# Psy-Fer/SquiggleKit

Hardware: AMD Instinct MI355X
Metric: reads/sec MotifSeq DTW (4k-sample read x 200-sample motif) (higher is better)
Workload: dtype f64 results; u32 fixed-point screening

## Files before the change

squigglekit_amd/csrc/sk_prepw_dev.h:

```cpp
#pragma once
#include "sk_common.h"

namespace {

typedef short i16x2 __attribute__((ext_vector_type(2)));

__device__ __forceinline__ unsigned clamp_pk_i16(unsigned q, unsigned lo2, unsigned hi2)
{
    const i16x2 x = __builtin_bit_cast(i16x2, q);
    const i16x2 c = __builtin_elementwise_min(__builtin_elementwise_max(x, __builtin_bit_cast(i16x2, lo2)),
                                              __builtin_bit_cast(i16x2, hi2));
    return __builtin_bit_cast(unsigned, c);
}

__device__ __forceinline__ int wave_incl_scan(int v)
{
    v += __builtin_amdgcn_update_dpp(0, v, 0x111, 0xF, 0xF, false);
    v += __builtin_amdgcn_update_dpp(0, v, 0x112, 0xF, 0xF, false);
    v += __builtin_amdgcn_update_dpp(0, v, 0x114, 0xF, 0xF, false);
    v += __builtin_amdgcn_update_dpp(0, v, 0x118, 0xF, 0xF, false);
    v += __builtin_amdgcn_update_dpp(0, v, 0x142, 0xA, 0xF, false);
    v += __builtin_amdgcn_update_dpp(0, v, 0x143, 0xC, 0xF, false);
    return v;
}
// ... 46 lines not shown
    const unsigned long long own2 = __ballot(local > 0 && k2 >= pre && k2 < pre + local);
    b1 = bcast_from(i1, own1 ? (int)__builtin_ctzll(own1) : 0);
    b2 = bcast_from(i2, own2 ? (int)__builtin_ctzll(own2) : 0);
}

struct prepw_env {
    unsigned *hist;
    int lo, hi, nbins, nb4;
    int hb0;
    bool in_vec, out_vec;
    unsigned lo2, hi2;
};

template <int NQ>
__device__ __forceinline__ prepw_env prepw_setup(unsigned *hist, int lane, int lo, int hi, int vec_ok)
{
    prepw_env e;
    e.hist = hist; e.lo = lo; e.hi = hi;
    e.nbins = hi - lo - 1;
    e.nb4 = (e.nbins + 3) & ~3;
    e.hb0 = lane * 4 * NQ;
    e.in_vec = (vec_ok & 1) != 0; e.out_vec = (vec_ok & 2) != 0;
    const int lo1 = max(lo + 1, -32768), hi1 = min(hi - 1, 32767);
    e.lo2 = (unsigned)(lo1 & 0xffff) * 0x10001u; e.hi2 = (unsigned)(hi1 & 0xffff) * 0x10001u;
#pragma unroll
    for (int j = 0; j < NQ; j++)
        if (e.hb0 + 4 * j < e.nb4) *(uint4 *)(hist + e.hb0 + 4 * j) = make_uint4(0u, 0u, 0u, 0u);
    return e;
}

template <int NQ>
__device__ __forceinline__ sk_prep prepw_read(const prepw_env &E, const int16_t *__restrict__ sig, int64_t stride,
                                              const int32_t *__restrict__ len, int r, int lane,
                                              int16_t *__restrict__ comp, sk_prep *__restrict__ prep)
{
    unsigned *const hist = E.hist;
    unsigned *const hist_v = hist - (E.lo + 1);
    const int lo = E.lo, hi = E.hi, nbins = E.nbins, nb4 = E.nb4, hb0 = E.hb0;
    const bool in_vec = E.in_vec, out_vec = E.out_vec;
    const unsigned lo2 = E.lo2, hi2 = E.hi2;
    auto load8 = [&](const int16_t *row, int M, int i0, unsigned (&q)[4]) {
        if (in_vec && i0 + 8 <= M) {
            const uint4 t = *(const uint4 *)(row + i0);
            q[0] = t.x; q[1] = t.y; q[2] = t.z; q[3] = t.w;
        } else {
#pragma unroll
            for (int k = 0; k < 4; k++) {
                const unsigned a = (i0 + 2 * k < M) ? (unsigned short)row[i0 + 2 * k] : 0u;
                const unsigned b = (i0 + 2 * k + 1 < M) ? (unsigned short)row[i0 + 2 * k + 1] : 0u;
                q[k] = a | (b << 16);
            }
        }
    };
    {
        const int M = min(max(len[r], 0), (int)min(stride, (int64_t)0x7fffff00));
        const int16_t *row = sig + (int64_t)r * stride;
        int16_t *crow = comp + (int64_t)r * stride;

        int run = 0;
        {
            unsigned v[4], vn[4];
            load8(row, M, lane * 8, v);
            for (int base = 0; base < M; base += 512) {
                const int i0 = base + lane * 8;
                if (base + 512 < M) load8(row, M, i0 + 512, vn);
                unsigned changed = 0;
#pragma unroll
// ... 6 lines not shown
                } else {
                    unsigned keep = 0;
#pragma unroll
                    for (int k = 0; k < 8; k++) {
                        const int x = sample_of(v, k);
                        if (i0 + k < M && x > lo && x < hi) keep |= 1u << k;
                    }
                    const int cnt = __popc(keep);
                    const int inc = wave_incl_scan(cnt);
                    int o = run + inc - cnt;
#pragma unroll
                    for (int k = 0; k < 8; k++) {
                        if (keep & (1u << k)) {
                            const int x = sample_of(v, k);
                            crow[o++] = (int16_t)x;
                            atomicAdd(&hist_v[x], 1u);
                        }
                    }
                    run += bcast_from(inc, 63);
                }
#pragma unroll
                for (int k = 0; k < 4; k++) v[k] = vn[k];
            }
        }
        const int n = run;

        sk_prep pr;
        pr.n = n; pr.flags = 0; pr.center = 0.0; pr.scale = 1.0; pr.top = 0.0; pr.bot = 0.0;
        if (n == 0) {
            pr.flags = SK_FLAG_EMPTY;
            const double qnan = __builtin_nan("");
            pr.center = qnan; pr.scale = qnan; pr.top = qnan; pr.bot = qnan;
            if (lane == 0) prep[r] = pr;
            return pr;
        }

        unsigned cnt[4 * NQ];
#pragma unroll
        for (int j = 0; j < NQ; j++) {
            uint4 q = make_uint4(0u, 0u, 0u, 0u);
            if (hb0 + 4 * j < nb4) q = *(const uint4 *)(hist + hb0 + 4 * j);
            cnt[4 * j] = q.x; cnt[4 * j + 1] = q.y; cnt[4 * j + 2] = q.z; cnt[4 * j + 3] = q.w;
        }
        int b1, b2, pre_med;
        rank2<NQ>(cnt, lane, (n - 1) / 2, n / 2, b1, b2, &pre_med);
        const int med2 = (b1 + lo + 1) + (b2 + lo + 1);

        const int odd = med2 & 1;
        const int cl = ((med2 - odd) >> 1) - (lo + 1);
        const int cr = cl + odd;
        {
            int acc = pre_med;
#pragma unroll
            for (int j = 0; j < NQ; j++) {
                uint4 q;
                acc += (int)cnt[4 * j];     q.x = (unsigned)acc;
                acc += (int)cnt[4 * j + 1]; q.y = (unsigned)acc;
                acc += (int)cnt[4 * j + 2]; q.z = (unsigned)acc;
                acc += (int)cnt[4 * j + 3]; q.w = (unsigned)acc;
                if (hb0 + 4 * j < nb4) *(uint4 *)(hist + hb0 + 4 * j) = q;
            }
        }
        auto within = [&](int t) -> int {
            const int hi_i = min(cr + t, nbins - 1), lo_i = cl - t - 1;
            const int a = (int)hist[hi_i];
            const int b = (lo_i >= 0) ? (int)hist[max(lo_i, 0)] : 0;
            return a - b;
        };
        const int k1 = (n - 1) / 2, k2 = n / 2;
        const int step = (nbins + 63) >> 6;
        const int cend = within(lane * step + step - 1);
        const unsigned long long ge1 = __ballot(cend > k1), ge2 = __ballot(cend > k2);
        const int B1 = ge1 ? (int)__builtin_ctzll(ge1) : 63, B2 = ge2 ? (int)__builtin_ctzll(ge2) : 63;
        const int half = lane >> 5, li = lane & 31;
        const int tprobe = (half ? B2 : B1) * step + li;
        const int cin = within(tprobe);
        const unsigned long long hit = __ballot(li < step && cin > (half ? k2 : k1));
        const unsigned h1 = (unsigned)hit, h2 = (unsigned)(hit >> 32);
        const int t1 = B1 * step + (h1 ? (int)__builtin_ctz(h1) : step - 1);
// ... 227 lines not shown
```

squigglekit_amd/csrc/sk_runtime.hip:

```cpp
#include "sk_common.h"
#include <string>
#include <string.h>
#include <mutex>
#include <stdio.h>
#include <stdlib.h>
#include <string.h>

static thread_local char  g_err[512] = "";
static thread_local int   g_cur = -1;
static sk_ctx             g_ctx[SK_MAX_DEVICES];
static std::mutex         g_mu;
static std::recursive_mutex g_ctx_mu[SK_MAX_DEVICES];

int sk_fail(int code, const char *fmt, ...)
{
    va_list ap;
    va_start(ap, fmt);
    vsnprintf(g_err, sizeof g_err, fmt, ap);
    va_end(ap);
    return code;
}

sk_entry::sk_entry() : sk_entry(g_cur) {}

// ... 23 lines not shown
    (void)c;
    if (bytes <= b->cap) return SK_OK;
    if (b->p) { SK_HIP(hipFree(b->p)); b->p = nullptr; b->cap = 0; }
    size_t want = bytes + bytes / 8 + 256;
    hipError_t e = hipMalloc(&b->p, want);
    if (e != hipSuccess) {
        b->p = nullptr;
        return sk_fail(SK_ERR_NOMEM, "hipMalloc(%zu) failed: %s", want, hipGetErrorString(e));
    }
    b->cap = want;
    return SK_OK;
}

int sk_second_stream(sk_ctx *c)
{
    if (!c->stream2) {
        SK_HIP(hipStreamCreateWithFlags(&c->stream2, hipStreamNonBlocking));
        for (int i = 0; i < 9; i++) SK_HIP(hipEventCreateWithFlags(&c->ev_chunk[i], hipEventDisableTiming));
    }
    return SK_OK;
}

struct sk_tunable { const char *name, *test_values, *what; };
static const sk_tunable SK_TUNABLES[] = {
    {"SK_DTW_SCHEME",         "full exact2", "DTW scheme: full = one exact pass, exact2 = two exact passes (default: fixed-point screening + certified window)"},
    {"SK_DTW_QL",             "8 16 64",     "lanes per read of the screening scheme (default: by motif length and batch size)"},
    {"SK_DTW_NOFUSE",         "1",           "filter + medmad as their own kernel instead of the screening pass's prologue"},
    {"SK_DTW_FORCE_RETRY_PM", "100 1000",    "per-mille of reads sent through the exact retry whatever the window pass certified (sensitivity runs)"},
    {"SK_DTW_SPAN",           "150 300",     "look-back of the window pass in columns (one tier)"},
    {"SK_DTW_SPAN2",          "0 500",       "look-back of the window pass's second tier (0: none)"},
    {"SK_DTW_CK",             "64 256",      "steps between checkpoints of the screening pass (multiple of 64)"},
    {"SK_DTW_NOSORT",         "1",           "window passes take the reads in file order"},
    {"SK_DTW_NOHINT",         "1",           "no start hint: the plain screening sweep, every read's exact window looks back the same number of columns"},
    {"SK_DTW_HINT_MIN",       "1",           "the start hint is on for calls of at least this many reads (default 500000)"},
    {"SK_DTW_SORT_MIN",       "1",           "window passes sort chunks of at least this many reads"},
    {"SK_DTW_NO_EARLY",       "1",           "no early exact retry beside the window passes"},
    {"SK_DTW_NO_SIBLINGS",    "1",           "reads whose candidate columns fall into two clusters take the exact pass (no second window)"},
    {"SK_DTW_NOGUARD",        "1",           "screening scheme without its run-time guard (premise test in the window pass, audit, gated exact fallback): A/B cost runs"},
    {"SK_DTW_AUDIT_PERIOD",   "0 1 64",      "the audit re-runs one read in this many with the exact pass (default 4096; 0: no audit)"},
    {"SK_DTW_HOLE",           "qerr1 fma64 fma64x", "tests: a known precision hole put back (E = 1; the fma sample image for float64 reads, with / without the image-error guard) -- the guard has to notice and the records must not change"},
    {"SK_DTW_SCRATCH_MB",     "8 64",        "checkpoint scratch budget in MB (small values force many chunks)"},
    {"SK_DTW_NO_SMALL",       "1",           "small batches keep the batch lane layout"},
    {"SK_DTW_SMALL_MAX",      "0 100000",    "largest batch that spreads a read over 64 lanes"},
    {"SK_PREP_BLOCK",         "1",           "medmad statistics by the workgroup-per-read kernel"},
    {"SK_PREP_ROUNDS",        "1 3",         "grid rounds of the persistent statistics kernels"},
    {"SK_PREP_PERCU",         "1 2",         "workgroups per CU of the persistent statistics kernels"},
    {"SK_SEG_OLD",            "1",           "segmenter: numpy-order statistics kernels for every read"},
    {"SK_SEG_DELTA_SCALE",    "1e13",        "segmenter: certification margin multiplier (large: every read takes the numpy-order redo)"},
    {"SK_SEG_PA_F64",         "1",           "segmenter, raw reads through the pA conversion: expand to float64 and take the float64 kernels instead of the raw-domain kernel"},
    {"SK_SEG_NO_WG",          "1",           "segmenter, reads of 4 097 .. 65 536 samples: the wavefront-per-read statistics kernel (two looks at a read) instead of the workgroup-per-read one"},
    {"SK_SEG_WG_ALL",         "1",           "segmenter: the workgroup-per-read statistics kernel for every row of 4 097 .. 65 536 samples (default: where it is faster)"},
    {"SK_SEG_OCC",            "7 8",         "segmenter statistics kernel: waves per SIMD the registers are sized for"},
    {"SK_SEG_CHUNKS",         "2 8",         "segmenter: chunks of a large batch (walk of one beside the statistics of the next)"},
    {"SK_WALK_GENERAL",       "1",           "segmenter walk: general step (corrector test live)"},
    {"SK_WALK_SYNC",          "1",           "segmenter walk: run hopping with the 64 lanes of a wavefront on the same word (k_seg_walk3)"},
    {"SK_WALK_OWNPASS",       "1",           "segmenter walk: finds the quiet stretches and anchors in a pass of its own instead of taking the statistics kernel's hints"},
    {"SK_WALK_NOJUMP",        "1",           "segmenter walk: every run is hopped through, no jumps between the stretches of quiet entries"},
    {"SK_WALK_NOWAVE",        "1",           "segmenter walk: a lane per read also for long rows / small batches (no wavefront-per-read walk)"},
    {"SK_WALK_WAVE_MAXREADS", "0 1000000",   "segmenter walk: batches of up to this many reads take the wavefront-per-read walk (default: 16384, 131072 for rows beyond 4 096 samples)"},
    {"SK_DRNA_STEP",          "1",           "dRNA_segmenter, both branches: the per-sample scans instead of the scans by runs / by transitions"},
    {"SK_ROLL_TWO_KERNELS",   "1",           "dRNA_segmenter rolling-mean branch: filter kernel + prefix sums through HBM instead of the one-look kernel (prefix sums in LDS)"},
    {"SK_ROLL_ONE_LOOK",      "1",           "dRNA_segmenter rolling-mean branch: the workgroup-per-read kernel in numpy's order for every read instead of the streaming kernel with certified thresholds"},
    {"SK_ROLL_DELTA_SCALE",   "1e13",        "dRNA_segmenter rolling-mean branch: multiplier of the certification margin (large: every read is redone in numpy's order)"},
    {"SK_HITS_ROW_BYTES",     "1000000",     "hit lists: bytes of the last-row buffer (12 B per column and read; default 2 GiB; small values force many chunks of reads)"},
    {"SK_PANEL_EXACT",        "1",           "motif panel: the one-grid exact kernel also for long windows over many reads (default: those take the screening scheme, one launch set per motif)"},
    {"SK_PATH_LDS_BYTES",     "0",           "alignment paths: bytes of direction words a hit may keep in LDS (default and most 25600; 0: every hit takes the scratch tier)"},
// ... 308 lines not shown
```

squigglekit_amd/csrc/sk_sdtwq.hip:

```cpp
#include "sk_sdtw_dev.h"
#include "sk_prepw_dev.h"
#include <math.h>
#include <stdlib.h>
#include <string.h>
#include <vector>

#ifndef SK_SDTWQ_FEED
#define SK_SDTWQ_FEED 0
#define SK_SDTWQ_MAIN 1
#endif

namespace {

template <int R>
__device__ __forceinline__ void qcolumn(const unsigned (&old)[R], unsigned (&nw)[R], const unsigned (&xq)[R],
                                        unsigned yq, unsigned dg, unsigned up)
{
    constexpr int R4 = R & ~3;
#pragma unroll
    for (int k = 0; k < R4; k += 4) {
        asm("v_min3_u32 %0, %12, %4, %13\n\t"
            "v_sad_u32 %0, %8, %14, %0 clamp\n\t"
            "v_min3_u32 %1, %4, %5, %0\n\t"
            "v_sad_u32 %1, %9, %14, %1 clamp\n\t"
// ... 98 lines not shown
    const unsigned *ls = a.lsum + (int64_t)(r - a.read0) * (a.nck + 1) * L + l;
    const unsigned thr = (b > QINF - 2u * a.qerr) ? QINF : b + 2u * a.qerr;
    int hs = 0x7fffffff;
    for (int cc = jlo / a.ck; cc <= min(a.nck, (jhi + L - 1) / a.ck); cc++) {
        if (ls[(int64_t)cc * L] > thr) continue;
        const int j0 = cc * a.ck + l - (L - 1);
        for (int q = 0; q < a.ck / L; q++) {
            const int j = j0 + q * L;
            if (j < jlo || j > jhi) continue;
            const unsigned w = lastq[j + L];
            if (w > thr) continue;
            const int gj = j >> HINT_G;
            const int gs = gj - (int)((unsigned)(gj - (int)(w & HINT_MASK)) & HINT_MASK);
            hs = min(hs, max(gs, 0) << HINT_G);
        }
    }
#pragma unroll
    for (int d = 1; d < L; d <<= 1) hs = min(hs, __shfl_xor(hs, d));
    return hs;
}

#ifndef SK_Q_WAVES
#define SK_Q_WAVES(R) 4
#endif
#ifdef SK_SDTWQ_HINT
#define SK_Q_KERNEL k_sdtw_qh
#define SK_P_KERNEL k_sdtw_ph
constexpr bool HINT = true;
#else
#define SK_Q_KERNEL k_sdtw_q
#define SK_P_KERNEL k_sdtw_p
constexpr bool HINT = false;
#endif
template <int L, int R, int FEED, bool P0>
__global__ __launch_bounds__(256) __attribute__((amdgpu_waves_per_eu(SK_Q_WAVES(R), 8)))
void SK_Q_KERNEL(const sdtw_kargs a)
{
    static_assert(L == 8 || L == 16 || L == 64, "lanes per read");
    static_assert(!HINT || (FEED == SK_FEED_I16 && L <= (1 << HINT_G) && (1 << HINT_G) % L == 0),
                  "tagged sweep: int16 feed, a block of L steps inside one granule");
    constexpr int G = 64 / L;
    constexpr int CKH = (R + 3) / 2;
    constexpr int U = (L < 16) ? L : 16;

    const int lane = threadIdx.x & 63;
    const int wave = blockIdx.x * (blockDim.x >> 6) + (threadIdx.x >> 6);
    const int g = lane / L, l = lane % L;
    int slot = wave * G + g;
    const bool live = slot < a.nreads;
    if (!live) slot = a.nreads - 1;
    const int r = a.read0 + slot;
    const bool timer = a.clk && blockIdx.x == 0 && threadIdx.x < 64;
    unsigned long long tc0 = 0, tr0 = 0;
    if (timer) { tc0 = __builtin_amdgcn_s_memtime(); tr0 = __builtin_amdgcn_s_memrealtime(); }

    extern __shared__ __align__(16) unsigned char lds_dyn[];
    __shared__ __align__(16) unsigned lds_all[4][5 * 64];
    int n;
    double center = 0.0, scale = 1.0;
    const int16_t *s16 = nullptr;
    const double  *s64 = nullptr;
    if constexpr (FEED == SK_FEED_I16) {
        if (a.fz_raw) {
            unsigned *wlds = (unsigned *)lds_dyn + (size_t)(threadIdx.x >> 6) * a.lds_wave_words;
            n = 0;
            if (a.fz_mode == 0) {
                const prepw_env E = prepw_setup<5>(wlds, lane, a.fz_lo, a.fz_hi, a.fz_vec);
                for (int gg = 0; gg < G; gg++) {
                    if (wave * G + gg >= a.nreads) break;
                    const sk_prep pr = prepw_read<5>(E, a.fz_raw, a.stride, a.fz_len, a.read0 + wave * G + gg, lane,
                                                     (int16_t *)a.samples, (sk_prep *)a.prep);
                    if (g == gg) { n = pr.n; center = pr.center; scale = pr.scale; }
                }
            } else {
                const zs_env E = zs_setup((int16_t *)wlds, (double *)lds_all[threadIdx.x >> 6], a.fz_lo, a.fz_hi, a.fz_vec);
#pragma unroll 1
                for (int gg = 0; gg < G; gg++) {
                    if (wave * G + gg >= a.nreads) break;
                    const sk_prep pr = zs_read(E, a.fz_raw, a.stride, a.fz_len, a.read0 + wave * G + gg, lane,
                                               (int16_t *)a.samples, (sk_prep *)a.prep);
                    if (g == gg) { n = pr.n; center = pr.center; scale = pr.scale; }
                    __builtin_amdgcn_wave_barrier();
                }
            }
            __builtin_amdgcn_fence(__ATOMIC_RELEASE, "workgroup");
            __builtin_amdgcn_fence(__ATOMIC_ACQUIRE, "workgroup");
        } else {
            const sk_prep pr = a.prep[r];
            n = pr.n; center = pr.center; scale = pr.scale;
        }
        s16 = (const int16_t *)a.samples + (int64_t)r * a.stride;
    } else if constexpr (FEED == SK_FEED_F64_NORM) {
        const sk_prep pr = a.prep[r];
        n = pr.n; center = pr.center; scale = pr.scale;
        s64 = (const double *)(((pr.flags & SK_IFLAG_INPLACE) && a.samples_raw) ? a.samples_raw : a.samples) + a.off[r];
    } else {
        n = (int)(a.off[r + 1] - a.off[r]);
        s64 = (const double *)a.samples + a.off[r];
    }
    if (!live) n = 0;
    const double inv_scale = 1.0 / scale;

    int nsteps = (n > 0) ? n - 1 + L : 0;
#pragma unroll
    for (int d = L; d < 64; d <<= 1) nsteps = max(nsteps, __shfl_xor(nsteps, d));
// ... 7 lines not shown
    const unsigned notfirst = (l == 0) ? 0u : 0xffffffffu;
    [[maybe_unused]] unsigned tagv = 0;

    unsigned Da[R], Db[R];
#pragma unroll
    for (int k = 0; k < R; k++) { Da[k] = QINF; Db[k] = QINF; }
    unsigned botq = (R == 1 && l == 0 && shortlane) ? 0u : QINF;
    unsigned diagq = (l == 0) ? 0u : QINF;
    int bad = 0;
    if constexpr (FEED == SK_FEED_F64_NORM) {
        if (live && (a.prep[r].flags & SK_FLAG_RECENTRE)) bad = 1;
    }
    unsigned qmin = QINF;
    unsigned smin = QINF;

    const int nlast = max(n - 1, 0);
    if (n == 0) { s16 = (const int16_t *)a.xlayq; s64 = (const double *)a.xlayq; }
    auto loadraw = [&](int idx) {
        if constexpr (FEED == SK_FEED_I16) return (int)s16[min(idx, nlast)];
        else                               return s64[min(idx, nlast)];
    };
    const double qa = inv_scale * QSCALE, qb = -center * qa;
    const bool fma64 = FEED == SK_FEED_F64_NORM && a.hole >= SK_HOLE_FMA64;
    if (live && n > 0) {
        double imgerr = 0.0;
        if (FEED == SK_FEED_I16 || fma64)            imgerr = 3.8e-7 + fabs(center) * qa * 1.2e-16;
        else if constexpr (FEED == SK_FEED_F64_NORM) imgerr = 5.7e-7;
        const bool rej = !(imgerr * (double)(HINT ? a.qplen : a.qerr) <= 1.0) && a.hole != SK_HOLE_FMA64_UNGUARDED;
        if (rej) {
            bad = 1;
            if (l == 0 && a.guard) atomicAdd(&a.guard[SK_GUARD_IMGREJ], 1);
        }
    }
    auto toq = [&](auto raw_, int idx) -> unsigned {
        const double raw = (double)raw_;
        double t;
        if constexpr (FEED == SK_FEED_I16)           t = __builtin_fma(raw, qa, qb);
        else if constexpr (FEED == SK_FEED_F64_NORM) t = fma64 ? __builtin_fma(raw, qa, qb) : (raw - center) * qa;
        else                                         t = raw * QSCALE;
        const bool ok = fabs(t) < QLIM * QSCALE;
        unsigned q = (unsigned)__double2loint(t + 6755399441055744.0) ^ 0x80000000u;
        if constexpr (HINT) q &= ~HINT_MASK;
        const bool in = idx < n;
        bad |= (in && !ok) ? 1 : 0;
        return (in && ok) ? q : QINF;
    };

    const unsigned smask = shortlane ? 0xffffffffu : 0u;
    unsigned *lastq = a.lastq + (int64_t)(r - a.read0) * a.lq_stride;
    unsigned *ybuf = lds_all[threadIdx.x >> 6] + g * 5 * L;
    unsigned *dump = ybuf + 3 * L;
    unsigned *ibuf = (unsigned *)lds_dyn + (size_t)(threadIdx.x >> 6) * a.lds_wave_words + g * a.ck;
    int ioff = 0;
    unsigned gmin = QINF;
    ybuf[L + l] = QINF;
    unsigned F = toq(loadraw(l), l);
    auto step = [&](const unsigned (&old)[R], unsigned (&nw)[R], unsigned yq, unsigned *hslot) {
        unsigned upq;
        if constexpr (HINT) upq = shrtag<L>(botq, tagv);
        else                upq = shr0<L>(botq, notfirst);
        qcolumn<R>(old, nw, xq, yq, diagq, upq);
        diagq = upq;
        if constexpr (P0)          botq = nw[R - 1];
        else if constexpr (R >= 2) asm("v_bitop3_b32 %0, %1, %2, %3 bitop3:0xe4" : "=v"(botq) : "v"(nw[R - 2]), "v"(nw[R - 1]), "v"(smask));
        else                       asm("v_bitop3_b32 %0, %1, %2, %3 bitop3:0xe4" : "=v"(botq) : "v"(upq), "v"(nw[0]), "v"(smask));
        *hslot = nw[R - 1];
    };
    auto flush = [&](int c, int nb) {
        unsigned im = smin;
#pragma unroll
        for (int d = 1; d < L; d <<= 1) im = min(im, (unsigned)__shfl_xor((int)im, d));
        const unsigned lim = (gmin > QINF - 2u * a.qerr) ? QINF : gmin + 2u * a.qerr;
        const bool keep = live && im <= lim;
        gmin = min(gmin, im);
        if (keep) {
            unsigned *dst = lastq + (int64_t)c * a.ck + l + 1;
            for (int q = 0; q < nb; q++) dst[q * L] = ibuf[q * L + l];
        }
// ... 220 lines not shown
            }
            const unsigned Fnext = toq(t0 + L + l);
            const unsigned *yr;
            if (pb & 1) { ybuf[L + l] = Fq; yr = ybuf + L - l; }
            else        { ybuf[l] = Fq; ybuf[2 * L + l] = Fq; yr = ybuf + 2 * L - l; }
#pragma unroll 1
            for (int q = 0; q < L; q += 2) {
                const unsigned y0 = yr[q], y1 = yr[q + 1];
                qstep(Qs, Qn, y0);
                qstep(Qn, Qs, y1);
            }
            Fq = Fnext;
        }
    }
    if (c0 > 0 && npre == 0) load_ckpt();
    tbase += npre * L;

    if (live) {
        if (c0 > 0) {
            unsigned *ws = a.wstate + ((int64_t)slot * L + l) * CKW;
#pragma unroll
            for (int k = 0; k < R; k++) ws[k] = Qs[k];
            ws[R] = botq; ws[R + 1] = diagq;
        }
        if (l == 0) {
            wrec w;
            w.tbase = tbase; w.jlo = jlo; w.jhi = jhi;
            w.flags = (screened ? 1 : 0) | (c0 > 0 ? 2 : 0) | clustered;
            ((wrec *)a.wrec)[slot] = w;
        }
    }
}

template <int L, int R, int FEED>
__global__ __launch_bounds__(256) __attribute__((amdgpu_waves_per_eu(R <= 13 ? 4 : (R <= 26 ? 3 : 2), 8)))
void k_sdtw_w(const sdtw_kargs a)
{
    constexpr int G = 64 / L;
    constexpr bool XLDS = R > 16;
    constexpr int SHR = (L == 64) ? DPP_WAVE_SHR1 : DPP_ROW_SHR1;
    constexpr int CKW = R + 2;
    constexpr int U = (L < 16) ? L : 8;
    const double INF = __builtin_huge_val();

    const int lane = threadIdx.x & 63;
    const int wave = blockIdx.x * (blockDim.x >> 6) + (threadIdx.x >> 6);
    const int g = lane / L, l = lane % L;
    int slot = wave * G + g;
    int nreads = a.nreads;
    if (a.wl_count) {
        nreads = min(*a.wl_count, a.nreads);
        if (nreads <= 0) return;
    }
    const bool live = slot < nreads;
    if (!live) slot = nreads - 1;
    const int r = a.tier2 == 2 ? ((const sibrec *)a.sib)[slot].r : a.wl_list ? a.wl_list[slot] : a.read0 + slot;

    int n, flags = 0;
    double center = 0.0, scale = 1.0;
    const int16_t *s16 = nullptr;
    const double  *s64 = nullptr;
    if constexpr (FEED == SK_FEED_I16) {
        const sk_prep pr = a.prep[r];
        n = pr.n; flags = pr.flags & SK_FLAG_PUBLIC; center = pr.center; scale = pr.scale;
        s16 = (const int16_t *)a.samples + (int64_t)r * a.stride;
    } else if constexpr (FEED == SK_FEED_F64_NORM) {
        const sk_prep pr = a.prep[r];
        n = pr.n; flags = pr.flags & SK_FLAG_PUBLIC; center = pr.center; scale = pr.scale;
        s64 = (const double *)(((pr.flags & SK_IFLAG_INPLACE) && a.samples_raw) ? a.samples_raw : a.samples) + a.off[r];
    } else {
// ... 88 lines not shown
#pragma unroll
            for (int q = 0; q < U; q++) {
                const int t = tbase + blk * L + qq + q;
                const double y = yv[q];
                double upD;  int upS;
                if constexpr (L >= 16) {
                    upD = dpp_f64<SHR>(0.0, botD);
                    upS = dpp_i32<SHR>(t + 1, botS);
                } else {
                    const unsigned lo = shr0<L>((unsigned)__double2loint(botD), notfirst);
                    const unsigned hi = shr0<L>((unsigned)__double2hiint(botD), notfirst);
                    upD = __hiloint2double((int)hi, (int)lo);
                    upS = (int)(shr0<L>((unsigned)botS, notfirst) | (first & (unsigned)(t + 1)));
                }
                double dgD = diagD;  int dgS = diagS;
                double uD = upD;     int uS = upS;
#pragma unroll
                for (int k = 0; k < R; k++) {
                    const double lfD = D[k];  const int lfS = S[k];
                    const double xk = XLDS ? xl[k] : x[k];
                    const double c = fabs(xk - y);
                    const bool lt1 = lfD < dgD;
                    const double m1 = vmin(lfD, dgD);
                    const int    s1 = lt1 ? lfS : dgS;
                    const bool lt2 = uD < m1;
                    const double m = vmin(uD, m1);
                    const int    s = lt2 ? uS : s1;
                    const double nd = c + m;
                    dgD = lfD;  dgS = lfS;
                    D[k] = nd;  S[k] = s;
                    uD = nd;    uS = s;
                }
                diagD = upD;  diagS = upS;
                if constexpr (R >= 2) {
                    botD = shortlane ? D[R - 2] : D[R - 1];
                    botS = shortlane ? S[R - 2] : S[R - 1];
                } else {
                    botD = shortlane ? upD : D[0];
                    botS = shortlane ? upS : S[0];
                }
                if (blk * L + qq + q >= s0) {
                    const int j = t - l;
                    if (j >= jlo && j <= jhi && D[R - 1] < best) { best = D[R - 1]; bestS = S[R - 1]; bestJ = j; }
                }
            }
        }
        F = Fnext;
    }

    auto premise_holds = [&](double bestD, int j) -> bool {
        if (!a.guard) return true;
        const unsigned lq = a.lastq[(int64_t)(r - a.read0) * a.lq_stride + j + L];
        const unsigned bq = (unsigned)a.qflag[r - a.read0];
        const double u = bestD * QSCALE, e = (double)a.qerr;
        const double e2 = (rec.flags & 4) ? 3.0 * e : e;
        const bool ok = fabs(u - (double)lq) <= e && u <= (double)bq + e2;
        if (!ok) { atomicAdd(&a.guard[SK_GUARD_VIOL], 1); atomicAdd(&a.guard[SK_GUARD_ALARM], 1); }
        return ok;
    };
    if (live && l == L - 1) {
        sk_hit h;
        h.n = n; h.flags = flags;
        const bool forced = a.force_retry && (((unsigned)r * 2654435761u) >> 22) < (unsigned)a.force_retry;
        bool certified = false;
        if (a.tier2 == 2) {
            h.dist = best; h.start = bestS; h.end = bestJ;
            h.n = (n > 0 && screened && bestS >= 0 && !forced && premise_holds(best, bestJ)) ? 1 : 0;
            a.sib_out[slot] = h;
        } else if (n <= 0) {
            h.dist = __builtin_nan(""); h.start = -1; h.end = -1;
            a.out[r] = h;
        } else if (screened && bestS >= 0 && !forced && (certified = premise_holds(best, bestJ))) {
            h.dist = best; h.start = bestS; h.end = bestJ;
            a.out[r] = h;
        } else if (!screened && a.early_cnt && !a.tier2) {
        } else {
            h.dist = __builtin_nan(""); h.start = -1; h.end = -1;
            a.out[r] = h;
            const bool violated = screened && bestS >= 0 && !forced && !certified;
            if (screened && a.soft && !forced && !violated) a.soft[atomicAdd(a.soft_cnt, 1)] = r;
            else                                            a.retry[atomicAdd(a.retry_cnt, 1)] = r;
        }
    }
}

typedef void (*sdtw_fn)(const sdtw_kargs);

template <int L, int FEED, int WHICH>
sdtw_fn pick_r(int R)
{
#ifndef SK_SDTWQ_HINT
#define SK_KERNEL(RR) (WHICH == 0 ? (sdtw_fn)SK_Q_KERNEL<L, RR, FEED, false> :     \
                       WHICH == 3 ? (sdtw_fn)SK_Q_KERNEL<L, RR, FEED, (RR >= 2)> : \
                       WHICH == 1 ? (sdtw_fn)SK_P_KERNEL<L, RR, FEED> : (sdtw_fn)k_sdtw_w<L, RR, FEED>)
#else
#define SK_KERNEL(RR) (WHICH == 0 ? (sdtw_fn)SK_Q_KERNEL<L, RR, FEED, false> :     \
                       WHICH == 3 ? (sdtw_fn)SK_Q_KERNEL<L, RR, FEED, (RR >= 2)> : (sdtw_fn)SK_P_KERNEL<L, RR, FEED>)
#endif
    switch (R) { SK_R_CASES_1_16(SK_KERNEL) }
    if constexpr (L != 64) {
        switch (R) { SK_R_CASES_17_32(SK_KERNEL) }
    }
#undef SK_KERNEL
    return nullptr;
}

template <int WHICH, int FEED>
sdtw_fn pick_l(int L, int R)
{
    if (L == 8)  return pick_r<8, FEED, WHICH>(R);
    if (L == 16) return pick_r<16, FEED, WHICH>(R);
#ifndef SK_SDTWQ_HINT
    return pick_r<64, FEED, WHICH>(R);
#else
    return nullptr;
#endif
}

}

#if defined(SK_SDTWQ_HINT)
void *sk_sdtwq_pick_hint(int which, int L, int R)
#elif SK_SDTWQ_FEED == 0
void *sk_sdtwq_pick_feed0(int which, int L, int R)
#elif SK_SDTWQ_FEED == 1
void *sk_sdtwq_pick_feed1(int which, int L, int R)
#else
void *sk_sdtwq_pick_feed2(int which, int L, int R)
#endif
{
    switch (which) {
    case 0: return (void *)pick_l<0, SK_SDTWQ_FEED>(L, R);
    case 1: return (void *)pick_l<1, SK_SDTWQ_FEED>(L, R);
    case 3: return (void *)pick_l<3, SK_SDTWQ_FEED>(L, R);
#ifndef SK_SDTWQ_HINT
    default: return (void *)pick_l<2, SK_SDTWQ_FEED>(L, R);
#else
    default: return nullptr;
#endif
    }
}

#ifdef SK_SDTWQ_MAIN
void *sk_sdtwq_pick_feed1(int which, int L, int R);
void *sk_sdtwq_pick_feed2(int which, int L, int R);
void *sk_sdtwq_pick_hint(int which, int L, int R);

static void screen_layout(int N, int64_t nreads, int64_t maxlen, int *L, int *R)
{
    int l = (N <= 8 * 32 && nreads >= (maxlen > 8192 ? 65536 : 49152)) ? 8 : (N <= 16 * 32) ? 16 : 64;
    if (const char *e = sk_tune("SK_DTW_QL")) {
        const int v = atoi(e);
        if ((v == 8 && N <= 8 * 32) || (v == 16 && N <= 16 * 32) || v == 64) l = v;
    }
    *L = l;
    *R = (N + l - 1) / l;
}

constexpr int ORDER_BINS = 1024;

struct order_args {
    const wrec    *rec;
    const int32_t *qflag;
    int nreads, read0, span, ck, nck, L, wmax;
    int hint;
    int32_t *hist;
    int32_t *order;
};

__device__ __forceinline__ int order_key(const order_args &a, int i)
{
    const wrec q = a.rec[i];
    const unsigned b = (unsigned)a.qflag[i];
    if (!((b < QSAFE) && (q.jhi >= q.jlo) && (q.jhi - q.jlo <= a.wmax))) return ORDER_BINS - 1;
    const int tx = a.hint ? min(max(q.tbase, 0), q.jlo) : max(0, q.jlo - a.span);
    int c0 = tx / a.ck;
    if (c0 > a.nck) c0 = a.nck;
    const int npre = c0 > 0 ? (tx - c0 * a.ck) / a.L : 0;
    const int tbase = c0 * a.ck + npre * a.L;
// ... 111 lines not shown
    int64_t chunk;
    while (true) {
        chunk = sk_dtw_chunk_reads(per_read, a->nreads);
        rc = sk_reserve(c, &c->ckpt, (size_t)chunk * (size_t)(nck > 0 ? nck : 1) * ck_bytes);
        if (!rc) rc = sk_reserve(c, &c->lastq, (size_t)chunk * lq_stride * sizeof(unsigned));
        if (!rc) rc = sk_reserve(c, &c->wstate, (size_t)chunk * state_bytes);
        if (!rc) rc = sk_reserve(c, &c->lsum, (size_t)chunk * (size_t)(nck + 1) * L * sizeof(unsigned));
        if (rc != SK_ERR_NOMEM || chunk <= 1024) break;
        sk_dtw_scratch_shrink(0);
    }
    if (rc) return rc;
    if ((rc = sk_reserve(c, &c->qflag, (size_t)chunk * sizeof(int32_t)))) return rc;
    if ((rc = sk_reserve(c, &c->wrec, (size_t)chunk * sizeof(wrec)))) return rc;
    if ((rc = sk_reserve(c, &c->wrecq, (size_t)chunk * sizeof(wrec)))) return rc;
    int sort_min = 32768;
    if (const char *e = sk_tune("SK_DTW_SORT_MIN")) { const int v = atoi(e); if (v > 0) sort_min = v; }
    const bool sorted = chunk >= sort_min && sk_tune("SK_DTW_NOSORT") == nullptr;
    if (sorted && (rc = sk_reserve(c, &c->order, ((size_t)chunk + ORDER_BINS) * sizeof(int32_t)))) return rc;
    const bool tiers = span2 > span;
    if (tiers && (rc = sk_reserve(c, &c->wsoft, ((size_t)chunk + 1) * sizeof(int32_t)))) return rc;
    const bool siblings = sk_tune("SK_DTW_NO_SIBLINGS") == nullptr;
    const int sib_cap = (int)(chunk / 64 + 1024);
    if (siblings) {
        if ((rc = sk_reserve(c, &c->sib, 16 + (size_t)sib_cap * sizeof(sibrec)))) return rc;
        if ((rc = sk_reserve(c, &c->sibout, (size_t)sib_cap * sizeof(sk_hit)))) return rc;
        if ((rc = sk_reserve(c, &c->sibstate, (size_t)sib_cap * (state_bytes + sizeof(wrec))))) return rc;
        if (c->stream3 && !c->ev_s[0])
            for (int i = 0; i < 2; i++) SK_HIP(hipEventCreateWithFlags(&c->ev_s[i], hipEventDisableTiming));
    }

    typedef void *(*pick_fn)(int, int, int);
    const pick_fn pk = a->feed == SK_FEED_I16 ? (pick_fn)sk_sdtwq_pick_feed0
                     : a->feed == SK_FEED_F64_NORM ? (pick_fn)sk_sdtwq_pick_feed1 : (pick_fn)sk_sdtwq_pick_feed2;
    sdtw_fn fq = (sdtw_fn)pk(P == 0 ? 3 : 0, L, R), fp = (sdtw_fn)pk(1, L, R), fw = (sdtw_fn)pk(2, L, R);
    const int64_t plen = (int64_t)N + maxlen + 2;
    int64_t hint_min = HINT_MIN_READS;
    if (const char *e = sk_tune("SK_DTW_HINT_MIN")) { const int v = atoi(e); if (v > 0) hint_min = v; }
    const bool hint = a->feed == SK_FEED_I16 && (L == 8 || L == 16) && plen <= HINT_MAX_PLEN && R <= HINT_MAX_R &&
                      a->nreads >= hint_min && sk_tune("SK_DTW_NOHINT") == nullptr;
    sdtw_fn fp1 = fp;
    if (hint) { fq = (sdtw_fn)sk_sdtwq_pick_hint(P == 0 ? 3 : 0, L, R); fp1 = (sdtw_fn)sk_sdtwq_pick_hint(1, L, R); }
    if (!fq || !fp || !fp1 || !fw) return sk_fail(SK_ERR_UNSUPPORTED, "no screening kernel for L=%d R=%d", L, R);

    sdtw_kargs k = kargs_of(a);
    k.xlay = (const double *)c->motifw.p; k.xlayq = (const unsigned *)c->motifq.p; k.P = P; k.out = a->out;
    k.nck = nck; k.ck = ck; k.span = span; k.retry = d_retry; k.retry_cnt = d_retry_cnt;
    k.ckq = (unsigned *)c->ckpt.p; k.lastq = (unsigned *)c->lastq.p; k.lq_stride = (int64_t)lq_stride;
    k.qflag = (int32_t *)c->qflag.p; k.lsum = (unsigned *)c->lsum.p;
    k.wstate = (unsigned *)c->wstate.p; k.wrec = c->wrec.p; k.wrec_q = c->wrecq.p;
    k.early_cnt = d_early_cnt; k.early = d_early;
    k.qplen = (unsigned)plen;
    k.qerr = hint ? ((unsigned)plen << HINT_T) + HINT_MASK : (unsigned)plen;
    k.wmax = 4 * ck;
    k.lds_wave_words = (64 / L) * ck;
    k.guard = sk_tune("SK_DTW_NOGUARD") ? nullptr : (int32_t *)c->dtwcnt.p + 8;
    k.wsteps = (unsigned long long *)((char *)c->dtwcnt.p + 64);
    if (const char *e = sk_tune("SK_DTW_HOLE")) {
        k.hole = strcmp(e, "qerr1") == 0 ? SK_HOLE_QERR1 : strcmp(e, "fma64") == 0 ? SK_HOLE_FMA64
               : strcmp(e, "fma64x") == 0 ? SK_HOLE_FMA64_UNGUARDED : SK_HOLE_NONE;
        if (k.hole == SK_HOLE_QERR1) k.qerr = 1;
    }
    if (const char *e = sk_tune("SK_DTW_FORCE_RETRY_PM")) {
        const int pm = atoi(e);
        if (pm > 0) k.force_retry = pm >= 1000 ? 1024 : (pm * 1024 + 999) / 1000;
    }

    size_t fz_lds = 0;
    const sk_prep_fuse fz = a->fuse ? *a->fuse : sk_prep_fuse();
    if (a->fuse) {
        const int need = fz.mode == SK_PREP_ZSCALE ? (int)((a->stride * 2 + 15) / 16 * 4) : (((fz.hi - fz.lo - 1) + 3) & ~3);
        if (need > k.lds_wave_words) k.lds_wave_words = need;
    }
    fz_lds = (size_t)4 * (size_t)k.lds_wave_words * sizeof(unsigned);
    if (fz_lds + 5 * 1024 > 64 * 1024)
// ... 99 lines not shown
```

Measured before the change: 17.48 million.

## Hoist fixed-point range test to per-read value range from fused prologue

The fused int16 filter+medmad prologue now reports each read's min and max sample value, taken from the histogram. The screening kernel checks the fixed-point overflow bound once per read on those two ends, so the per-sample range test and bad-flag update leave the hot conversion. A window-kernel variant for P==0 also reads the bottom row directly instead of selecting on shortlane. This adds new template instantiations and a separate compile unit, and the per-read test is only valid because quantization is monotone in the raw value.

```diff
diff --git a/squigglekit_amd/csrc/sk_prepw_dev.h b/squigglekit_amd/csrc/sk_prepw_dev.h
--- a/squigglekit_amd/csrc/sk_prepw_dev.h
+++ b/squigglekit_amd/csrc/sk_prepw_dev.h
@@ -102,7 +102,8 @@
 template <int NQ>
 __device__ __forceinline__ sk_prep prepw_read(const prepw_env &E, const int16_t *__restrict__ sig, int64_t stride,
                                               const int32_t *__restrict__ len, int r, int lane,
-                                              int16_t *__restrict__ comp, sk_prep *__restrict__ prep)
+                                              int16_t *__restrict__ comp, sk_prep *__restrict__ prep,
+                                              int (*vrange)[2] = nullptr)
 {
     unsigned *const hist = E.hist;
     unsigned *const hist_v = hist - (E.lo + 1);
@@ -175,6 +176,7 @@
             const double qnan = __builtin_nan("");
             pr.center = qnan; pr.scale = qnan; pr.top = qnan; pr.bot = qnan;
             if (lane == 0) prep[r] = pr;
+            if (vrange) { (*vrange)[0] = 0; (*vrange)[1] = 0; }
             return pr;
         }
 
@@ -188,6 +190,16 @@
         int b1, b2, pre_med;
         rank2<NQ>(cnt, lane, (n - 1) / 2, n / 2, b1, b2, &pre_med);
         const int med2 = (b1 + lo + 1) + (b2 + lo + 1);
+        if (vrange) {
+            int first = 4 * NQ, last = -1;
+#pragma unroll
+            for (int i = 4 * NQ - 1; i >= 0; i--) if (cnt[i]) first = i;
+#pragma unroll
+            for (int i = 0; i < 4 * NQ; i++) if (cnt[i]) last = i;
+            const unsigned long long have = __ballot(last >= 0);
+            (*vrange)[0] = bcast_from(hb0 + first, (int)__builtin_ctzll(have)) + lo + 1;
+            (*vrange)[1] = bcast_from(hb0 + last, 63 - (int)__builtin_clzll(have)) + lo + 1;
+        }
 
         const int odd = med2 & 1;
         const int cl = ((med2 - odd) >> 1) - (lo + 1);
diff --git a/squigglekit_amd/csrc/sk_runtime.hip b/squigglekit_amd/csrc/sk_runtime.hip
--- a/squigglekit_amd/csrc/sk_runtime.hip
+++ b/squigglekit_amd/csrc/sk_runtime.hip
@@ -79,6 +79,7 @@
     {"SK_DTW_CK",             "64 256",      "steps between checkpoints of the screening pass (multiple of 64)"},
     {"SK_DTW_NOSORT",         "1",           "window passes take the reads in file order"},
     {"SK_DTW_NOHINT",         "1",           "no start hint: the plain screening sweep, every read's exact window looks back the same number of columns"},
+    {"SK_DTW_RANGE_PER_SAMPLE", "1",         "screening sweep behind the fused filter + medmad prologue: the fixed-point range test on every sample (default there: once per read, on the ends of its value range)"},
     {"SK_DTW_HINT_MIN",       "1",           "the start hint is on for calls of at least this many reads (default 500000)"},
     {"SK_DTW_SORT_MIN",       "1",           "window passes sort chunks of at least this many reads"},
     {"SK_DTW_NO_EARLY",       "1",           "no early exact retry beside the window passes"},
diff --git a/squigglekit_amd/csrc/sk_sdtwq.hip b/squigglekit_amd/csrc/sk_sdtwq.hip
--- a/squigglekit_amd/csrc/sk_sdtwq.hip
+++ b/squigglekit_amd/csrc/sk_sdtwq.hip
@@ -154,11 +154,15 @@
 #define SK_P_KERNEL k_sdtw_p
 constexpr bool HINT = false;
 #endif
-template <int L, int R, int FEED, bool P0>
+constexpr int SK_FEED_VARIANT = 4;
+template <int L, int R, int FEEDX, bool P0>
 __global__ __launch_bounds__(256) __attribute__((amdgpu_waves_per_eu(SK_Q_WAVES(R), 8)))
 void SK_Q_KERNEL(const sdtw_kargs a)
 {
+    constexpr bool RNG = (FEEDX & SK_FEED_VARIANT) != 0;
+    constexpr int FEED = FEEDX & ~SK_FEED_VARIANT;
     static_assert(L == 8 || L == 16 || L == 64, "lanes per read");
+    static_assert(!RNG || FEED == SK_FEED_I16, "per-read range test: the fused int16 prologue hands over the value range");
     static_assert(!HINT || (FEED == SK_FEED_I16 && L <= (1 << HINT_G) && (1 << HINT_G) % L == 0),
                   "tagged sweep: int16 feed, a block of L steps inside one granule");
     constexpr int G = 64 / L;
@@ -180,6 +184,7 @@
     __shared__ __align__(16) unsigned lds_all[4][5 * 64];
     int n;
     double center = 0.0, scale = 1.0;
+    [[maybe_unused]] int vlo = 0, vhi = 0;
     const int16_t *s16 = nullptr;
     const double  *s64 = nullptr;
     if constexpr (FEED == SK_FEED_I16) {
@@ -190,9 +195,10 @@
                 const prepw_env E = prepw_setup<5>(wlds, lane, a.fz_lo, a.fz_hi, a.fz_vec);
                 for (int gg = 0; gg < G; gg++) {
                     if (wave * G + gg >= a.nreads) break;
+                    int vr[2] = {0, 0};
                     const sk_prep pr = prepw_read<5>(E, a.fz_raw, a.stride, a.fz_len, a.read0 + wave * G + gg, lane,
-                                                     (int16_t *)a.samples, (sk_prep *)a.prep);
-                    if (g == gg) { n = pr.n; center = pr.center; scale = pr.scale; }
+                                                     (int16_t *)a.samples, (sk_prep *)a.prep, RNG ? &vr : nullptr);
+                    if (g == gg) { n = pr.n; center = pr.center; scale = pr.scale; vlo = vr[0]; vhi = vr[1]; }
                 }
             } else {
                 const zs_env E = zs_setup((int16_t *)wlds, (double *)lds_all[threadIdx.x >> 6], a.fz_lo, a.fz_hi, a.fz_vec);
@@ -266,18 +272,31 @@
             if (l == 0 && a.guard) atomicAdd(&a.guard[SK_GUARD_IMGREJ], 1);
         }
     }
+    if constexpr (RNG) {
+        if (n > 0) {
+            const double tlo = __builtin_fma((double)vlo, qa, qb), thi = __builtin_fma((double)vhi, qa, qb);
+            if (!(fabs(tlo) < QLIM * QSCALE && fabs(thi) < QLIM * QSCALE)) bad = 1;
+        }
+    }
     auto toq = [&](auto raw_, int idx) -> unsigned {
         const double raw = (double)raw_;
         double t;
-        if constexpr (FEED == SK_FEED_I16)           t = __builtin_fma(raw, qa, qb);
-        else if constexpr (FEED == SK_FEED_F64_NORM) t = fma64 ? __builtin_fma(raw, qa, qb) : (raw - center) * qa;
-        else                                         t = raw * QSCALE;
-        const bool ok = fabs(t) < QLIM * QSCALE;
-        unsigned q = (unsigned)__double2loint(t + 6755399441055744.0) ^ 0x80000000u;
-        if constexpr (HINT) q &= ~HINT_MASK;
-        const bool in = idx < n;
-        bad |= (in && !ok) ? 1 : 0;
-        return (in && ok) ? q : QINF;
+        if constexpr (RNG) {
+            t = __builtin_fma(raw, qa, qb);
+            unsigned q = (unsigned)__double2loint(t + (6755399441055744.0 + 2147483648.0));
+            if constexpr (HINT) q &= ~HINT_MASK;
+            return (idx < n) ? q : QINF;
+        } else {
+            if constexpr (FEED == SK_FEED_I16)           t = __builtin_fma(raw, qa, qb);
+            else if constexpr (FEED == SK_FEED_F64_NORM) t = fma64 ? __builtin_fma(raw, qa, qb) : (raw - center) * qa;
+            else                                         t = raw * QSCALE;
+            const bool ok = fabs(t) < QLIM * QSCALE;
+            unsigned q = (unsigned)__double2loint(t + 6755399441055744.0) ^ 0x80000000u;
+            if constexpr (HINT) q &= ~HINT_MASK;
+            const bool in = idx < n;
+            bad |= (in && !ok) ? 1 : 0;
+            return (in && ok) ? q : QINF;
+        }
     };
 
     const unsigned smask = shortlane ? 0xffffffffu : 0u;
@@ -564,10 +583,12 @@
     }
 }
 
-template <int L, int R, int FEED>
+template <int L, int R, int FEEDX>
 __global__ __launch_bounds__(256) __attribute__((amdgpu_waves_per_eu(R <= 13 ? 4 : (R <= 26 ? 3 : 2), 8)))
 void k_sdtw_w(const sdtw_kargs a)
 {
+    constexpr bool P0 = (FEEDX & SK_FEED_VARIANT) != 0;
+    constexpr int FEED = FEEDX & ~SK_FEED_VARIANT;
     constexpr int G = 64 / L;
     constexpr bool XLDS = R > 16;
     constexpr int SHR = (L == 64) ? DPP_WAVE_SHR1 : DPP_ROW_SHR1;
@@ -722,7 +743,10 @@
                     uD = nd;    uS = s;
                 }
                 diagD = upD;  diagS = upS;
-                if constexpr (R >= 2) {
+                if constexpr (P0) {
+                    botD = D[R - 1];
+                    botS = S[R - 1];
+                } else if constexpr (R >= 2) {
                     botD = shortlane ? D[R - 2] : D[R - 1];
                     botS = shortlane ? S[R - 2] : S[R - 1];
                 } else {
@@ -776,6 +800,7 @@
 
 typedef void (*sdtw_fn)(const sdtw_kargs);
 
+#ifndef SK_SDTWQ_VAR
 template <int L, int FEED, int WHICH>
 sdtw_fn pick_r(int R)
 {
@@ -795,6 +820,49 @@
     return nullptr;
 }
 
+#endif
+
+#if defined(SK_SDTWQ_VAR) || defined(SK_SDTWQ_HINT)
+template <int L, int FEED, int WHICH>
+sdtw_fn pick_r_var(int R)
+{
+    if constexpr (WHICH != 6 && FEED == SK_FEED_I16) {
+#define SK_KERNEL_Q(RR) (WHICH == 4 ? (sdtw_fn)SK_Q_KERNEL<L, RR, FEED | SK_FEED_VARIANT, false> \
+                                    : (sdtw_fn)SK_Q_KERNEL<L, RR, FEED | SK_FEED_VARIANT, (RR >= 2)>)
+        switch (R) { SK_R_CASES_1_16(SK_KERNEL_Q) }
+#ifdef SK_SDTWQ_HINT
+        static_assert(HINT_MAX_R == 25, "the cases below");
+        switch (R) {
+        case 17: return SK_KERNEL_Q(17); case 18: return SK_KERNEL_Q(18); case 19: return SK_KERNEL_Q(19);
+        case 20: return SK_KERNEL_Q(20); case 21: return SK_KERNEL_Q(21); case 22: return SK_KERNEL_Q(22);
+        case 23: return SK_KERNEL_Q(23); case 24: return SK_KERNEL_Q(24); case 25: return SK_KERNEL_Q(25);
+        }
+#else
+        switch (R) { SK_R_CASES_17_32(SK_KERNEL_Q) }
+#endif
+#undef SK_KERNEL_Q
+    }
+#ifdef SK_SDTWQ_VAR
+#define SK_KERNEL_W(RR) (RR >= 2 ? (sdtw_fn)k_sdtw_w<L, RR, FEED | SK_FEED_VARIANT> : (sdtw_fn)k_sdtw_w<L, RR, FEED>)
+    if constexpr (WHICH == 6) {
+        switch (R) { SK_R_CASES_1_16(SK_KERNEL_W) }
+        switch (R) { SK_R_CASES_17_32(SK_KERNEL_W) }
+    }
+#undef SK_KERNEL_W
+#endif
+    return nullptr;
+}
+
+template <int WHICH, int FEED>
+sdtw_fn pick_l_var(int L, int R)
+{
+    if (L == 8)  return pick_r_var<8, FEED, WHICH>(R);
+    if (L == 16) return pick_r_var<16, FEED, WHICH>(R);
+    return nullptr;
+}
+#endif
+
+#ifndef SK_SDTWQ_VAR
 template <int WHICH, int FEED>
 sdtw_fn pick_l(int L, int R)
 {
@@ -807,8 +875,23 @@
 #endif
 }
 
-}
-
+#endif
+
+}
+
+#if defined(SK_SDTWQ_VAR)
+void *sk_sdtwq_pick_var(int which, int feed, int L, int R)
+{
+    switch (which) {
+    case 4: return feed == SK_FEED_I16 ? (void *)pick_l_var<4, SK_FEED_I16>(L, R) : nullptr;
+    case 5: return feed == SK_FEED_I16 ? (void *)pick_l_var<5, SK_FEED_I16>(L, R) : nullptr;
+    case 6: return feed == SK_FEED_I16 ? (void *)pick_l_var<6, SK_FEED_I16>(L, R)
+                 : feed == SK_FEED_F64_NORM ? (void *)pick_l_var<6, SK_FEED_F64_NORM>(L, R)
+                 : (void *)pick_l_var<6, SK_FEED_F64_RAW>(L, R);
+    default: return nullptr;
+    }
+}
+#else
 #if defined(SK_SDTWQ_HINT)
 void *sk_sdtwq_pick_hint(int which, int L, int R)
 #elif SK_SDTWQ_FEED == 0
@@ -826,15 +909,19 @@
 #ifndef SK_SDTWQ_HINT
     default: return (void *)pick_l<2, SK_SDTWQ_FEED>(L, R);
 #else
+    case 4: return (void *)pick_l_var<4, SK_SDTWQ_FEED>(L, R);
+    case 5: return (void *)pick_l_var<5, SK_SDTWQ_FEED>(L, R);
     default: return nullptr;
 #endif
     }
 }
+#endif
 
 #ifdef SK_SDTWQ_MAIN
 void *sk_sdtwq_pick_feed1(int which, int L, int R);
 void *sk_sdtwq_pick_feed2(int which, int L, int R);
 void *sk_sdtwq_pick_hint(int which, int L, int R);
+void *sk_sdtwq_pick_var(int which, int feed, int L, int R);
 
 static void screen_layout(int N, int64_t nreads, int64_t maxlen, int *L, int *R)
 {
@@ -1012,14 +1099,18 @@
     typedef void *(*pick_fn)(int, int, int);
     const pick_fn pk = a->feed == SK_FEED_I16 ? (pick_fn)sk_sdtwq_pick_feed0
                      : a->feed == SK_FEED_F64_NORM ? (pick_fn)sk_sdtwq_pick_feed1 : (pick_fn)sk_sdtwq_pick_feed2;
-    sdtw_fn fq = (sdtw_fn)pk(P == 0 ? 3 : 0, L, R), fp = (sdtw_fn)pk(1, L, R), fw = (sdtw_fn)pk(2, L, R);
+    const bool rng = a->feed == SK_FEED_I16 && a->fuse && a->fuse->mode != SK_PREP_ZSCALE && (L == 8 || L == 16) &&
+                     sk_tune("SK_DTW_RANGE_PER_SAMPLE") == nullptr;
+    const int wq = P == 0 ? 3 : 0;
+    sdtw_fn fq = rng ? (sdtw_fn)sk_sdtwq_pick_var(wq + 2, a->feed, L, R) : (sdtw_fn)pk(wq, L, R), fp = (sdtw_fn)pk(1, L, R);
+    sdtw_fn fw = (P == 0 && R >= 2 && L != 64) ? (sdtw_fn)sk_sdtwq_pick_var(6, a->feed, L, R) : (sdtw_fn)pk(2, L, R);
     const int64_t plen = (int64_t)N + maxlen + 2;
     int64_t hint_min = HINT_MIN_READS;
     if (const char *e = sk_tune("SK_DTW_HINT_MIN")) { const int v = atoi(e); if (v > 0) hint_min = v; }
     const bool hint = a->feed == SK_FEED_I16 && (L == 8 || L == 16) && plen <= HINT_MAX_PLEN && R <= HINT_MAX_R &&
                       a->nreads >= hint_min && sk_tune("SK_DTW_NOHINT") == nullptr;
     sdtw_fn fp1 = fp;
-    if (hint) { fq = (sdtw_fn)sk_sdtwq_pick_hint(P == 0 ? 3 : 0, L, R); fp1 = (sdtw_fn)sk_sdtwq_pick_hint(1, L, R); }
+    if (hint) { fq = (sdtw_fn)sk_sdtwq_pick_hint(rng ? wq + 2 : wq, L, R); fp1 = (sdtw_fn)sk_sdtwq_pick_hint(1, L, R); }
     if (!fq || !fp || !fp1 || !fw) return sk_fail(SK_ERR_UNSUPPORTED, "no screening kernel for L=%d R=%d", L, R);
 
     sdtw_kargs k = kargs_of(a);
diff --git a/squigglekit_amd/csrc/sk_sdtwq_var.hip b/squigglekit_amd/csrc/sk_sdtwq_var.hip
--- /dev/null
+++ b/squigglekit_amd/csrc/sk_sdtwq_var.hip
@@ -0,0 +1,3 @@
+#define SK_SDTWQ_FEED 0
+#define SK_SDTWQ_VAR 1
+#include "sk_sdtwq.hip"
```

Result: no change. 17.63 million, median of 6 (+0.8%).
